# MrTornado24/FENeRF

Hardware: NVIDIA H100
Metric: rendered faces/sec at 128px x 24 samples/ray (higher is better)
Workload: dtype f16 operands / f32 accumulate (wgmma) + f32 refinement

## Files before the change

fenerf_b200/csrc/siren_fast.cu:

```cuda
#include "siren_fast.cuh"

namespace fn {

int siren_fast_label_launch(const void* args, int blocks, cudaStream_t st);
int siren_fast_hd_launch(const void* args, int blocks, bool label_film, cudaStream_t st);
int siren_fast_grid_launch(const void* args, int blocks, cudaStream_t st);
int siren_fast_bridge_launch(const void* args, int blocks, cudaStream_t st);
int siren_fast_debug_launch(const void* args, int blocks, bool label_film, bool feature_head, int variant, cudaStream_t st);

namespace {

std::atomic<int> g_variant{0};
unsigned long long* g_trace = nullptr;
int g_trace_ctas = 0;

bool build_loads(const FnLayout& L, FastArgs& A, bool sigma_only) {
    A.n_loads = 0;
    auto push = [&](size_t src, uint32_t bytes) {
        if (A.n_loads < MAX_LOADS) A.loads[A.n_loads] = Load{(uint32_t)src, bytes};
        ++A.n_loads;
    };
    push(L.first_img, 2 * CHUNK);
    if (L.grid_trunk) push(L.first_img_lo, 2 * CHUNK);
    for (int l = 0; l < L.n_hidden; ++l) {
        if (l == L.trunk_hidden) {
            push(L.head_img, 4 * HEAD_CHUNK);
            if (sigma_only) return A.n_loads <= MAX_LOADS;
        }
        if (L.bridge && l == L.color0) {
            push(L.color0_ximg, 2 * CHUNK);
            continue;
        }
        push(L.hid_img[l], 2 * CHUNK);
        push(L.hid_img[l] + 2 * CHUNK, 2 * CHUNK);
        if (l == L.label_layer) push(L.label.img, (uint32_t)FN_HEAD_IMG_BYTES(L.label.img_rows));
        if (l == L.color0) push(L.color0_ximg, 2 * CHUNK);
        push(L.hid_img[l] + 4 * CHUNK, 2 * CHUNK);
        push(L.hid_img[l] + 6 * CHUNK, 2 * CHUNK);
    }
    push(L.rgb.img, (uint32_t)FN_HEAD_IMG_BYTES(L.rgb.img_rows));
    return A.n_loads <= MAX_LOADS;
}

}

int siren_fast_debug_variant(int variant, unsigned long long* trace, int trace_ctas) {
    FN_REQUIRE(variant >= 0 && variant <= 3, "unknown point-network variant %d", variant);
    FN_REQUIRE(variant < 2 || (trace && trace_ctas >= 1), "a timeline variant needs its trace buffer");
    g_trace = trace;
    g_trace_ctas = trace_ctas;
    g_variant.store(variant);
    return 0;
}

int siren_points_fast(const FnLayout& L, const unsigned char* packed, const float* points, const float* dirs, const float* film,
                      int batch, long long ppb, int dir_group, int lock_dirs, float* out, int sigma_only, cudaStream_t st,
                      float* sigma_out) {
    static_assert(sizeof(FastArgs) <= 4000, "kernel parameter block too large");
    static_assert(SMEM_TOTAL <= 232448, "one CTA per SM: 227 KB of shared memory");
    static_assert(FN_HEAD_IMG_BYTES(FN_FEAT) == SLOT_BYTES, "a feature-head image is one ring slot");
    const bool trunk_only = L.feature_head && sigma_only;
    const bool feature_head = L.feature_head && !trunk_only, label_film = L.label_film && !trunk_only;
    FN_REQUIRE(L.trunk_hidden >= 1 && L.n_hidden - L.color0 >= 1, "field needs >= 2 trunk and >= 1 colour layers");
    FN_REQUIRE(L.sigma_row < 32, "the fast path packs labels and sigma into one 32-column head (label_dim <= 31)");
    FN_REQUIRE(L.rgb.img < 0xFFFFFFFFull && L.label.img < 0xFFFFFFFFull && L.first_img_lo < 0xFFFFFFFFull,
               "packed weight images beyond 4 GB");
    FN_REQUIRE(((uintptr_t)film & 15) == 0, "the FiLM table must be 16-byte aligned");
    if (L.wo_dir && !sigma_only)
        return fail(FENERF_E_UNSUPPORTED, "FENERF_FIELD_WO_DIR: the wgmma colour branch is not accurate for this field (its "
                    "first colour layer amplifies the fp16 trunk's error to ~2e-2 in rgb); render it with "
                    "FENERF_PRECISION_EXACT or FENERF_PRECISION_SPLIT (the density alone runs in any precision)");
    FastArgs a;
    memset(&a, 0, sizeof(a));
    FN_REQUIRE(build_loads(L, a, sigma_only != 0), "field too deep for the weight stream");
    a.sigma_only = sigma_only ? 1 : 0;
    a.L = L; a.packed = packed; a.points = points; a.dirs = dirs; a.film = film; a.out = out; a.sigma_out = sigma_out;
    a.ppb = ppb; a.tiles_per_batch = (ppb + TILE - 1) / TILE; a.n_tiles = a.tiles_per_batch * batch;
    a.dir_group = dir_group < 1 ? 1 : dir_group; a.lock_dirs = lock_dirs;
    if (a.n_tiles <= 0) return 0;
    FN_REQUIRE(ppb % a.dir_group == 0, "points_per_batch %lld not a multiple of dir_group %d", ppb, a.dir_group);
    const long long n_pairs = (a.n_tiles + 1) / 2;
    const int blocks = (int)(n_pairs < (long long)num_sms() ? n_pairs : (long long)num_sms());
    if (const int variant = g_variant.load()) {
        FN_REQUIRE(!L.grid_trunk && !L.bridge,
                   "the debug point-network variants do not cover fields with the grid in the trunk or a bridge");
        a.trace = g_trace;
        a.trace_ctas = g_trace_ctas;
        return siren_fast_debug_launch(&a, blocks, label_film, feature_head, variant, st);
    }
    if (L.grid_trunk) return siren_fast_grid_launch(&a, blocks, st);
    if (L.bridge) return siren_fast_bridge_launch(&a, blocks, st);
    if (feature_head) return siren_fast_hd_launch(&a, blocks, label_film, st);
    if (label_film) return siren_fast_label_launch(&a, blocks, st);
    return launch<siren_fast_kernel<false>>("siren_fast_kernel", blocks, NTHREADS, SMEM_TOTAL, st, a);
}

}
```

fenerf_b200/csrc/siren_fast.cuh:

```cuda
#pragma once
#include "common.cuh"
#include "siren_common.cuh"
#include "sm90.cuh"

namespace fn {

namespace {

using namespace sm90;

constexpr int TILE = 64;
constexpr int NTHREADS = 384;
constexpr int PROD_WARP = 8;
constexpr int RING = 6;
constexpr uint32_t SLOT_BYTES = 32768;
constexpr int XSTRIDE = 72;
constexpr uint32_t SMEM_X = RING * SLOT_BYTES;
constexpr int FRING = 2;
constexpr uint32_t FILM_BYTES = 2 * FN_H * 4;
constexpr uint32_t SMEM_FILM = SMEM_X + 2 * TILE * XSTRIDE * 2;
constexpr uint32_t SMEM_BAR = SMEM_FILM + 2 * FRING * FILM_BYTES;
constexpr uint32_t SMEM_TOTAL = SMEM_BAR + 16 * RING + 16 + 16 * 2 * FRING;
constexpr uint32_t SMEM_XLO = SMEM_TOTAL;
constexpr int XLO_STRIDE = 32;
constexpr uint32_t SMEM_TOTAL_GRID = SMEM_XLO + 2 * TILE * XLO_STRIDE * 2;
constexpr int RING_SPLIT = 4;
constexpr uint32_t ALO_CHUNK = TILE * FN_KCHUNK * 2;
constexpr uint32_t ALO_BYTES = (FN_H / FN_KCHUNK) * ALO_CHUNK;
constexpr uint32_t SPLIT_SMEM_ALO = RING_SPLIT * SLOT_BYTES;
constexpr uint32_t SPLIT_SMEM_X = SPLIT_SMEM_ALO + 2 * ALO_BYTES;
constexpr uint32_t SPLIT_SMEM_FILM = SPLIT_SMEM_X + 2 * TILE * XSTRIDE * 2;
constexpr uint32_t SPLIT_SMEM_BAR = SPLIT_SMEM_FILM + 2 * FRING * FILM_BYTES;
constexpr uint32_t SPLIT_SMEM_XLO = SPLIT_SMEM_BAR + 16 * RING_SPLIT + 16 + 16 * 2 * FRING;
constexpr uint32_t SMEM_TOTAL_SPLIT = SPLIT_SMEM_XLO + 2 * TILE * XLO_STRIDE * 2;
constexpr int MAX_LOADS = 72;
constexpr int MAX_LOADS_SPLIT = 132;
constexpr uint32_t CHUNK = 16384;
constexpr uint32_t HEAD_CHUNK = 32 * 128;
constexpr uint32_t RGB_CHUNK = 8 * 128;
constexpr uint32_t FEAT_CHUNK = FN_FEAT * 128;
#ifndef FENERF_SOFT_SIN_EVERY
#define FENERF_SOFT_SIN_EVERY 0
#endif
constexpr int kSoftSinEvery = FENERF_SOFT_SIN_EVERY;
constexpr int kSoftSinSplit = 4;
constexpr int TRACE_CAP = 1024;
constexpr int TRACE_WARPS = 11;
enum TraceEvent {
    TR_PAIR = 1, TR_TURN_WAIT, TR_TURN_DONE, TR_ACQ_WAIT, TR_ACQ_DONE, TR_COMMIT, TR_MMA_DONE, TR_EPI_DONE,
    TR_FILM_WAIT, TR_FILM_DONE, TR_EMPTY_WAIT, TR_EMPTY_DONE,
};
enum TraceGroup { TG_FIRST = 0, TG_HIDDEN, TG_COLOR0, TG_TRUNK_HEAD, TG_LABEL_LAYER, TG_LABEL_HEAD, TG_OUT_HEAD };

__device__ __forceinline__ float soft_sinf(float a) {
    const float k = fmaf(a, 0.159154943f, 12582912.f);
    const float n = k - 12582912.f;
    float r = fmaf(-n, 6.28318548f, a);
    r = fmaf(-n, -1.74845553e-7f, r);
    const float r2 = r * r;
    float p = -2.041572245e-08f;
    p = fmaf(p, r2, 2.701100129e-06f);
    p = fmaf(p, r2, -1.980991656e-04f);
    p = fmaf(p, r2, 8.332454599e-03f);
    p = fmaf(p, r2, -1.666656137e-01f);
    p = fmaf(p, r2, 9.999996424e-01f);
    return r * p;
}

struct Load {
    uint32_t src;
    uint32_t bytes;
};

template <int kMaxLoads>
struct FastArgsT {
    Load loads[kMaxLoads];
    int n_loads;
    FnLayout L;
    const unsigned char* packed;
    const float* points;
    const float* dirs;
    const float* film;
    float* out;
    float* sigma_out;
    long long ppb, tiles_per_batch, n_tiles;
    int dir_group, lock_dirs;
    int sigma_only;
    unsigned long long* trace;
    int trace_ctas;
};
using FastArgs = FastArgsT<MAX_LOADS>;
using SplitArgs = FastArgsT<MAX_LOADS_SPLIT>;

__device__ __forceinline__ void wg_bar(int wg) { asm volatile("bar.sync %0, 128;" ::"r"(1 + wg) : "memory"); }

template <bool kLabelFilm, bool kFeatureHead = false, int kSoftSin = kSoftSinEvery, bool kTrace = false,
          bool kGridTrunk = false, bool kBridge = false, bool kSplit = false>
__global__ void __launch_bounds__(NTHREADS, 1)
    siren_fast_kernel(const __grid_constant__ FastArgsT<kSplit ? MAX_LOADS_SPLIT : MAX_LOADS> a) {
    constexpr int RING = kSplit ? RING_SPLIT : fn::RING;
    constexpr uint32_t SMEM_X = kSplit ? SPLIT_SMEM_X : fn::SMEM_X;
    constexpr uint32_t SMEM_FILM = kSplit ? SPLIT_SMEM_FILM : fn::SMEM_FILM;
    constexpr uint32_t SMEM_BAR = kSplit ? SPLIT_SMEM_BAR : fn::SMEM_BAR;
    constexpr uint32_t SMEM_XLO = kSplit ? SPLIT_SMEM_XLO : fn::SMEM_XLO;
    extern __shared__ __align__(1024) unsigned char smem[];
    const uint32_t sbase = smem_u32(smem);
    const int warp = threadIdx.x >> 5, lane = threadIdx.x & 31;
    const uint32_t bar_full = sbase + SMEM_BAR, bar_empty = bar_full + 8 * RING, bar_turn = bar_empty + 8 * RING;
    const uint32_t bar_ffull = bar_turn + 16, bar_fempty = bar_ffull + 8 * 2 * FRING;
    unsigned long long* tbuf = nullptr;
    uint32_t tn = 0;
    if constexpr (kTrace)
        if (lane == 0 && (int)blockIdx.x < a.trace_ctas) tbuf = a.trace + ((size_t)blockIdx.x * TRACE_WARPS + warp) * TRACE_CAP;
    auto trace = [&](int kind, int group = 0) {
        if constexpr (kTrace)
            if (tbuf && tn < TRACE_CAP)
                tbuf[tn++] = ((unsigned long long)kind << 56) | ((unsigned long long)group << 48) |
                             ((unsigned long long)clock64() & ((1ull << 48) - 1));
    };
    if (threadIdx.x == 0) {
        for (int i = 0; i < RING; ++i) {
            mbar_init(bar_full + 8 * i, 1);
            mbar_init(bar_empty + 8 * i, 8);
        }
        for (int g = 0; g < 2; ++g) mbar_init(bar_turn + 8 * g, 4);
        for (int e = 0; e < 2 * FRING; ++e) {
            mbar_init(bar_ffull + 8 * e, 32);
            mbar_init(bar_fempty + 8 * e, 4);
        }
        fence_barrier_init();
    }
    __syncthreads();
    const long long n_pairs = (a.n_tiles + 1) / 2;

    if (warp >= PROD_WARP) {
        asm volatile("setmaxnreg.dec.sync.aligned.u32 40;\n" ::: "memory");
        if (warp == PROD_WARP && lane == 0) {
            uint32_t it = 0;
            for (long long pair = blockIdx.x; pair < n_pairs; pair += gridDim.x)
                for (int i = 0; i < a.n_loads; ++i, ++it) {
                    const uint32_t slot = it % RING;
                    trace(TR_EMPTY_WAIT);
                    mbar_wait(bar_empty + 8 * slot, ((it / RING) & 1u) ^ 1u);
                    trace(TR_EMPTY_DONE);
                    mbar_arrive_expect_tx(bar_full + 8 * slot, a.loads[i].bytes);
                    bulk_g2s(sbase + slot * SLOT_BYTES, a.packed + a.loads[i].src, a.loads[i].bytes, bar_full + 8 * slot);
                }
        } else if (warp == PROD_WARP + 1 || warp == PROD_WARP + 2) {
            const int g = warp - PROD_WARP - 1;
            const int n_film = 1 + (a.sigma_only ? a.L.trunk_hidden : a.L.n_hidden);
            uint32_t it = 0;
            for (long long pair = blockIdx.x; pair < n_pairs; pair += gridDim.x) {
                const long long tile = pair * 2 + g;
                const long long b = tile < a.n_tiles ? tile / a.tiles_per_batch : 0;
                const float* film_b = a.film + (size_t)b * a.L.n_film * 2 * FN_H;
                for (int i = 0; i < n_film; ++i, ++it) {
                    const uint32_t e = g * FRING + it % FRING;
                    const float2* row = reinterpret_cast<const float2*>(film_b + (size_t)i * 2 * FN_H);
                    const float2* bias = reinterpret_cast<const float2*>(a.packed + (i == 0 ? a.L.first_b : a.L.hid_b[i - 1]));
                    float4* dst = reinterpret_cast<float4*>(smem + SMEM_FILM + e * FILM_BYTES);
                    trace(TR_EMPTY_WAIT);
                    mbar_wait(bar_fempty + 8 * e, ((it / FRING) & 1u) ^ 1u);
                    trace(TR_EMPTY_DONE);
#pragma unroll 1
                    for (int k = 0; k < FN_H / 64; ++k) {
                        const int cp = lane + 32 * k;
                        const float2 f = __ldg(row + cp), p = __ldg(row + FN_H / 2 + cp), bb = __ldg(bias + cp);
                        if constexpr (kSplit) {
                            const float us = __ldg(reinterpret_cast<const float*>(a.packed + a.L.split_scale) +
                                                   FN_SPLIT_SCALES + i);
                            dst[cp] = make_float4(f.x * us, f.y * us, fmaf(f.x, bb.x, p.x), fmaf(f.y, bb.y, p.y));
                        } else {
                            dst[cp] = make_float4(f.x, f.y, fmaf(f.x, bb.x, p.x), fmaf(f.y, bb.y, p.y));
                        }
                    }
                    mbar_arrive(bar_ffull + 8 * e);
                }
            }
        }
        return;
    }

    asm volatile("setmaxnreg.inc.sync.aligned.u32 232;\n" ::: "memory");
    const int wg = warp >> 2, q = lane & 3;
    const int tid = threadIdx.x & 127;
    const int r0 = (warp & 3) * 16 + (lane >> 2);
    const FnLayout& L = a.L;
    const int C = L.out_dim;
    const float* sigma_w = reinterpret_cast<const float*>(a.packed + L.sigma_w);
    const float* label_w = reinterpret_cast<const float*>(a.packed + L.label_w);
    const int trunk_labels = (kLabelFilm || kFeatureHead) ? 0 : L.trunk_labels;
    const int sigma_row = kFeatureHead ? FN_FEAT_SIGMA_ROW : L.sigma_row;
    const int rgb_rows = kFeatureHead ? FN_FEAT : L.rgb.w_rows;
    const int label_rows = kFeatureHead ? FN_FEAT : L.label.w_rows;
    __half* xs = reinterpret_cast<__half*>(smem + SMEM_X) + wg * TILE * XSTRIDE;
    uint32_t it = 0;
    auto acquire = [&](uint32_t& slot) -> uint32_t {
        slot = it % RING;
        trace(TR_ACQ_WAIT);
        mbar_wait(bar_full + 8 * slot, (it / RING) & 1u);
        trace(TR_ACQ_DONE);
        ++it;
        return sbase + slot * SLOT_BYTES;
    };
    auto release = [&](uint32_t slot) {
        __syncwarp();
        if (lane == 0) mbar_arrive(bar_empty + 8 * slot);
    };
    uint32_t turns = 0;
    uint32_t fit = 0;
    auto film_acquire = [&]() -> const float4* {
        const uint32_t e = wg * FRING + fit % FRING;
        trace(TR_FILM_WAIT);
        mbar_wait(bar_ffull + 8 * e, (fit / FRING) & 1u);
        trace(TR_FILM_DONE);
        return reinterpret_cast<const float4*>(smem + SMEM_FILM + e * FILM_BYTES);
    };
    auto film_release = [&]() {
        const uint32_t e = wg * FRING + fit % FRING;
        ++fit;
        __syncwarp();
        if (lane == 0) mbar_arrive(bar_fempty + 8 * e);
    };
    auto turn_begin = [&]() {
        trace(TR_TURN_WAIT);
        mbar_wait(bar_turn + 8 * wg, (turns & 1u) ^ (wg == 0 ? 1u : 0u));
        trace(TR_TURN_DONE);
    };
    auto turn_end = [&](int group) {
        trace(TR_COMMIT, group);
        ++turns;
        __syncwarp();
        if (lane == 0) mbar_arrive(bar_turn + 8 * (wg ^ 1));
    };
    auto xfrag = [&](int s, uint32_t (&f)[4]) {
        const __half* p = xs + r0 * XSTRIDE + 16 * s + 2 * q;
        f[0] = *reinterpret_cast<const uint32_t*>(p);
        f[1] = *reinterpret_cast<const uint32_t*>(p + 8 * XSTRIDE);
        f[2] = *reinterpret_cast<const uint32_t*>(p + 8);
        f[3] = *reinterpret_cast<const uint32_t*>(p + 8 * XSTRIDE + 8);
    };

    for (long long pair = blockIdx.x; pair < n_pairs; pair += gridDim.x) {
        const long long tile = pair * 2 + wg;
        const bool tile_ok = tile < a.n_tiles;
        const long long b = tile_ok ? tile / a.tiles_per_batch : 0;
        const long long p0 = tile_ok ? (tile % a.tiles_per_batch) * TILE : a.ppb;
        trace(TR_PAIR);

        wg_bar(wg);
        if (tid < TILE) {
            float pos[3] = {0.f, 0.f, 0.f}, dir[3] = {0.f, 0.f, 0.f};
            const long long pp = p0 + tid;
            const bool valid = pp < a.ppb;
            if (valid) {
                const long long ff = b * a.ppb + pp;
#pragma unroll
                for (int i = 0; i < 3; ++i) pos[i] = __fmul_rn(a.points[ff * 3 + i], L.input_scale);
                if (a.lock_dirs) dir[2] = -1.f;
                else {
                    const long long di = b * (a.ppb / a.dir_group) + pp / a.dir_group;
#pragma unroll
                    for (int i = 0; i < 3; ++i) dir[i] = a.dirs[di * 3 + i];
                }
            }
            __align__(16) __half slots[64];
#pragma unroll
            for (int i = 0; i < 64; ++i) slots[i] = __float2half_rn(0.f);
#pragma unroll
            for (int i = 0; i < 3; ++i) {
                __half hi, lo;
                split_f16(pos[i], hi, lo);
                slots[FN_SLOT_POS + i] = hi; slots[FN_SLOT_POS + 3 + i] = lo; slots[FN_SLOT_POS + 6 + i] = hi;
                split_f16(dir[i], hi, lo);
                slots[FN_SLOT_DIR + i] = hi; slots[FN_SLOT_DIR + 3 + i] = lo; slots[FN_SLOT_DIR + 6 + i] = hi;
            }
            if constexpr (kGridTrunk || kSplit) {
                __align__(16) __half lo[32];
#pragma unroll
                for (int i = 0; i < 32; ++i) lo[i] = __float2half_rn(0.f);
                if (valid && (kGridTrunk || (L.grid_channels > 0 && !a.sigma_only))) {
                    float feat[32];
                    grid_features32(reinterpret_cast<const float*>(a.packed + L.grid), L.grid_res, pos[0], pos[1], pos[2], feat);
#pragma unroll
                    for (int i = 0; i < 32; ++i) split_f16(feat[i], slots[FN_SLOT_FEAT + i], lo[i]);
                }
                __half* xlo = reinterpret_cast<__half*>(smem + SMEM_XLO) + (wg * TILE + tid) * XLO_STRIDE;
#pragma unroll
                for (int i = 0; i < 4; ++i) reinterpret_cast<uint4*>(xlo)[i] = reinterpret_cast<const uint4*>(lo)[i];
            } else if (L.grid_channels > 0 && valid && !a.sigma_only) {
                float feat[32];
                grid_features32_h(reinterpret_cast<const __half*>(a.packed + L.grid16), L.grid_res, pos[0], pos[1], pos[2], feat);
#pragma unroll
                for (int i = 0; i < 32; ++i) slots[FN_SLOT_FEAT + i] = __float2half_rn(feat[i]);
            }
#pragma unroll
            for (int i = 0; i < 8; ++i)
                reinterpret_cast<uint4*>(xs + tid * XSTRIDE)[i] = reinterpret_cast<const uint4*>(slots)[i];
        }
        wg_bar(wg);

        uint32_t act[16][4];
        uint32_t nxt[8][4];
        float d[64];
        auto film_epi = [&](const float4* fs, int h, uint32_t (&dst)[8][4]) {
#pragma unroll
            for (int j = 0; j < 16; ++j) {
                const float4 e = fs[64 * h + 4 * j + q];
                const bool soft = kSoftSin > 0 && j % (kSoftSin > 0 ? kSoftSin : 1) == kSoftSin - 1;
                auto sn = [soft](float x) { return soft ? soft_sinf(x) : __sinf(x); };
                dst[j >> 1][(j & 1) * 2] = pack_half2(sn(fmaf(e.x, d[4 * j], e.z)), sn(fmaf(e.y, d[4 * j + 1], e.w)));
                dst[j >> 1][(j & 1) * 2 + 1] = pack_half2(sn(fmaf(e.x, d[4 * j + 2], e.z)), sn(fmaf(e.y, d[4 * j + 3], e.w)));
            }
            trace(TR_EPI_DONE);
        };
        auto act_hi = [&]() -> uint32_t (&)[8][4] { return *reinterpret_cast<uint32_t (*)[8][4]>(&act[8]); };
        auto film_epi_split = [&](const float4* fs, int h, uint32_t (&dst)[8][4], uint32_t (&lo)[8][4]) {
#pragma unroll
            for (int j = 0; j < 16; ++j) {
                const float4 e = fs[64 * h + 4 * j + q];
#pragma unroll
                for (int rr = 0; rr < 2; ++rr) {
                    const float s0 = soft_sinf(fmaf(e.x, d[4 * j + 2 * rr], e.z));
                    const float s1 = soft_sinf(fmaf(e.y, d[4 * j + 2 * rr + 1], e.w));
                    const __half2 hi = __floats2half2_rn(s0, s1);
                    const float2 hf = __half22float2(hi);
                    dst[j >> 1][(j & 1) * 2 + rr] = *reinterpret_cast<const uint32_t*>(&hi);
                    lo[j >> 1][(j & 1) * 2 + rr] = pack_half2(s0 - hf.x, s1 - hf.y);
                }
            }
            trace(TR_EPI_DONE);
        };
        const uint32_t alo_base = sbase + SPLIT_SMEM_ALO + wg * ALO_BYTES;
        auto alo_desc = [&](int s) { return desc_kmajor(alo_base + (s >> 2) * ALO_CHUNK + 32 * (s & 3)); };
        auto alo_store = [&](const uint32_t (&lo0)[8][4], const uint32_t (&lo1)[8][4]) {
            wg_bar(wg);
            unsigned char* base = smem + SPLIT_SMEM_ALO + wg * ALO_BYTES;
#pragma unroll
            for (int h = 0; h < 2; ++h)
#pragma unroll
                for (int j = 0; j < 16; ++j) {
                    const int col = 128 * h + 8 * j + 2 * q;
#pragma unroll
                    for (int rr = 0; rr < 2; ++rr)
                        *reinterpret_cast<uint32_t*>(base + (col >> 6) * ALO_CHUNK + fn_sw128_offset(r0 + 8 * rr, col & 63)) =
                            (h ? lo1 : lo0)[j >> 1][(j & 1) * 2 + rr];
                }
            fence_async_smem();
            wg_bar(wg);
        };
        uint32_t lo0[8][4], lo1[8][4];

        {
            uint32_t xf[4], slot, slot_lo = 0, w_lo = 0;
            uint32_t xg[2][4], xl[2][4];
            const float4* fs = nullptr;
            xfrag(0, xf);
            if constexpr (kGridTrunk) {
                const __half* xlo = reinterpret_cast<const __half*>(smem + SMEM_XLO) + wg * TILE * XLO_STRIDE;
#pragma unroll
                for (int s = 0; s < 2; ++s) {
                    xfrag(2 + s, xg[s]);
                    const __half* p = xlo + r0 * XLO_STRIDE + 16 * s + 2 * q;
                    xl[s][0] = *reinterpret_cast<const uint32_t*>(p);
                    xl[s][1] = *reinterpret_cast<const uint32_t*>(p + 8 * XLO_STRIDE);
                    xl[s][2] = *reinterpret_cast<const uint32_t*>(p + 8);
                    xl[s][3] = *reinterpret_cast<const uint32_t*>(p + 8 * XLO_STRIDE + 8);
                }
            }
            const uint32_t w = acquire(slot);
            if constexpr (kGridTrunk) w_lo = acquire(slot_lo);
#pragma unroll
            for (int h = 0; h < 2; ++h) {
                turn_begin();
                wg_fence();
                mma_rs_n128(d, xf, desc_kmajor(w + h * CHUNK), 0u);
                if constexpr (kGridTrunk)
#pragma unroll
                    for (int s = 0; s < 2; ++s) {
                        mma_rs_n128(d, xg[s], desc_kmajor(w + h * CHUNK + 32 * (2 + s)), 1u);
                        mma_rs_n128(d, xl[s], desc_kmajor(w + h * CHUNK + 32 * (2 + s)), 1u);
                        mma_rs_n128(d, xg[s], desc_kmajor(w_lo + h * CHUNK + 32 * (2 + s)), 1u);
                    }
                wg_commit();
                turn_end(TG_FIRST);
                wg_wait<0>();
                trace(TR_MMA_DONE);
                fence_regs(d);
                fence_regs(xf);
                if constexpr (kGridTrunk) { fence_regs(xg); fence_regs(xl); }
                if (h == 0) fs = film_acquire();
                if constexpr (kSplit) {
                    if (h == 0) film_epi_split(fs, 0, nxt, lo0);
                    else film_epi_split(fs, 1, act_hi(), lo1);
                } else {
                    if (h == 0) film_epi(fs, 0, nxt);
                    else film_epi(fs, 1, act_hi());
                }
            }
            release(slot);
            if constexpr (kGridTrunk) release(slot_lo);
            film_release();
            if constexpr (kSplit) alo_store(lo0, lo1);
#pragma unroll
            for (int s = 0; s < 8; ++s)
#pragma unroll
                for (int i = 0; i < 4; ++i) act[s][i] = nxt[s][i];
        }

        bool stop = false;
        for (int l = 0; l < L.n_hidden && !stop; ++l) {
            if (l == L.trunk_hidden) {
                float dh[16];
                uint32_t slot, slot_lo = 0, w_lo = 0;
                const uint32_t w = acquire(slot);
                if constexpr (kSplit) w_lo = acquire(slot_lo);
                turn_begin();
                wg_fence();
#pragma unroll
                for (int c = 0; c < 4; ++c)
#pragma unroll
                    for (int k = 0; k < 4; ++k) mma_rs_n32(dh, act[4 * c + k], desc_kmajor(w + c * HEAD_CHUNK + 32 * k), (c | k) ? 1u : 0u);
                if constexpr (kSplit)
#pragma unroll
                    for (int c = 0; c < 4; ++c)
#pragma unroll
                        for (int k = 0; k < 4; ++k) {
                            mma_ss_n32(dh, alo_desc(4 * c + k), desc_kmajor(w + c * HEAD_CHUNK + 32 * k), 1u);
                            mma_rs_n32(dh, act[4 * c + k], desc_kmajor(w_lo + c * HEAD_CHUNK + 32 * k), 1u);
                        }
                wg_commit();
                turn_end(TG_TRUNK_HEAD);
                wg_wait<0>();
                trace(TR_MMA_DONE);
                fence_regs(dh);
                fence_regs(act);
                release(slot);
                if constexpr (kSplit) {
                    release(slot_lo);
                    const float us = __ldg(reinterpret_cast<const float*>(a.packed + L.split_scale) + FN_SPLIT_SCALES +
                                           L.n_hidden + 1);
#pragma unroll
                    for (int i = 0; i < 16; ++i) dh[i] *= us;
                }
                const float* lb = label_w + FENERF_MAX_LABEL * FN_H;
#pragma unroll
                for (int rr = 0; rr < 2; ++rr) {
                    const long long pnt = p0 + r0 + 8 * rr;
                    if (pnt >= a.ppb) continue;
                    const long long flat = b * a.ppb + pnt;
#pragma unroll
                    for (int i = 0; i < 4; ++i)
#pragma unroll
                        for (int e = 0; e < 2; ++e) {
                            const int o = 8 * i + 2 * q + e;
                            const float v = dh[4 * i + 2 * rr + e];
                            if (o < trunk_labels) {
                                if (!a.sigma_only) a.out[flat * C + o] = fmaf(v, __ldg(lb + FENERF_MAX_LABEL), __ldg(lb + o));
                            } else if (o == sigma_row && !(kBridge && L.bridge_res)) {
                                const float sig = v + __ldg(sigma_w + FN_H);
                                a.out[flat * C + (C - 1)] = sig;
                                if (a.sigma_out) a.sigma_out[flat] = sig;
                            }
                        }
                }
                if constexpr (kBridge) {
                    const float* bw = reinterpret_cast<const float*>(a.packed + L.bridge_w);
#pragma unroll
                    for (int rr = 0; rr < 2; ++rr) {
                        const float o0 = dh[2 * rr], o1 = dh[2 * rr + 1];
                        const float p2 = __shfl_xor_sync(0xffffffffu, o0, 1), p3 = __shfl_xor_sync(0xffffffffu, o1, 1);
                        if (q != 0) continue;
                        const long long pnt = p0 + r0 + 8 * rr;
                        float v[3] = {o1 + __ldg(bw + 3 * FN_H), p2 + __ldg(bw + 3 * FN_H + 1), p3 + __ldg(bw + 3 * FN_H + 2)};
                        if (L.bridge_res) {
                            if (pnt < a.ppb) {
                                const long long flat = b * a.ppb + pnt;
#pragma unroll
                                for (int j = 0; j < 3; ++j) v[j] += __fmul_rn(a.points[flat * 3 + j], L.input_scale);
                                float sig = __ldg(bw + 3 * FN_H + 6);
#pragma unroll
                                for (int j = 0; j < 3; ++j) sig = fmaf(__ldg(bw + 3 * FN_H + 3 + j), v[j], sig);
                                a.out[flat * C + (C - 1)] = sig;
                                if (a.sigma_out) a.sigma_out[flat] = sig;
                            }
                        }
                        if (!a.sigma_only) {
                            __half* row = xs + (r0 + 8 * rr) * XSTRIDE + FN_SLOT_FEAT;
#pragma unroll
                            for (int j = 0; j < 3; ++j) {
// ... 71 lines not shown
                    }
                    continue;
                }
            }
            const bool c0 = (l == L.color0);
            if constexpr (kSplit) {
                const bool grid = L.grid_channels > 0;
                const float4* fs = nullptr;
#pragma unroll
                for (int h = 0; h < 2; ++h) {
                    uint32_t sl[4], w[4];
#pragma unroll
                    for (int i = 0; i < 4; ++i) w[i] = acquire(sl[i]);
                    turn_begin();
                    wg_fence();
#pragma unroll
                    for (int s = 0; s < 16; ++s)
                        mma_rs_n128(d, act[s], desc_kmajor(w[s >> 3] + ((s >> 2) & 1) * CHUNK + 32 * (s & 3)), s ? 1u : 0u);
#pragma unroll
                    for (int s = 0; s < 16; ++s)
                        mma_ss_n128(d, alo_desc(s), desc_kmajor(w[s >> 3] + ((s >> 2) & 1) * CHUNK + 32 * (s & 3)), 1u);
#pragma unroll
                    for (int s = 0; s < 16; ++s)
                        mma_rs_n128(d, act[s], desc_kmajor(w[2 + (s >> 3)] + ((s >> 2) & 1) * CHUNK + 32 * (s & 3)), 1u);
                    wg_commit();
                    turn_end(c0 ? TG_COLOR0 : TG_HIDDEN);
                    wg_wait<0>();
                    trace(TR_MMA_DONE);
                    fence_regs(d);
                    fence_regs(act);
#pragma unroll
                    for (int i = 0; i < 4; ++i) release(sl[i]);
                    if (c0) {
                        uint32_t xf[3][4], xl[2][4], slot_x, slot_xl = 0, w_xl = 0;
#pragma unroll
                        for (int s = 0; s < 3; ++s) xfrag(1 + s, xf[s]);
                        const __half* xlo = reinterpret_cast<const __half*>(smem + SMEM_XLO) + wg * TILE * XLO_STRIDE;
#pragma unroll
                        for (int s = 0; s < 2; ++s) {
                            const __half* p = xlo + r0 * XLO_STRIDE + 16 * s + 2 * q;
                            xl[s][0] = *reinterpret_cast<const uint32_t*>(p);
                            xl[s][1] = *reinterpret_cast<const uint32_t*>(p + 8 * XLO_STRIDE);
                            xl[s][2] = *reinterpret_cast<const uint32_t*>(p + 8);
                            xl[s][3] = *reinterpret_cast<const uint32_t*>(p + 8 * XLO_STRIDE + 8);
                        }
                        const uint32_t w_x = acquire(slot_x);
                        if (grid) w_xl = acquire(slot_xl);
                        turn_begin();
                        wg_fence();
                        mma_rs_n128(d, xf[0], desc_kmajor(w_x + h * CHUNK + 32), 1u);
                        if (grid)
#pragma unroll
                            for (int s = 0; s < 2; ++s) {
                                const uint32_t off = h * CHUNK + 32 * (2 + s);
                                mma_rs_n128(d, xf[1 + s], desc_kmajor(w_x + off), 1u);
                                mma_rs_n128(d, xl[s], desc_kmajor(w_x + off), 1u);
                                mma_rs_n128(d, xf[1 + s], desc_kmajor(w_xl + off), 1u);
                            }
                        wg_commit();
                        turn_end(TG_COLOR0);
                        wg_wait<0>();
                        trace(TR_MMA_DONE);
                        fence_regs(d);
                        fence_regs(xf);
                        fence_regs(xl);
                        release(slot_x);
                        if (grid) release(slot_xl);
                    }
                    if (h == 0) fs = film_acquire();
                    if (h == 0) film_epi_split(fs, 0, nxt, lo0);
                    else film_epi_split(fs, 1, act_hi(), lo1);
                }
                film_release();
                alo_store(lo0, lo1);
#pragma unroll
                for (int s = 0; s < 8; ++s)
#pragma unroll
                    for (int i = 0; i < 4; ++i) act[s][i] = nxt[s][i];
                continue;
            }
            const bool narrow = kBridge && c0;
            const int nx = kBridge ? 2 : !kGridTrunk && L.grid_channels > 0 ? 3 : 1;
            uint32_t xf[3][4];
            if (c0)
#pragma unroll
                for (int s = 0; s < 3; ++s) xfrag(1 + s, xf[s]);
            uint32_t slot_x = 0, w_x = 0;
            const float4* fs = nullptr;
#pragma unroll
            for (int h = 0; h < 2; ++h) {
                uint32_t sl[2] = {0u, 0u};
                if (narrow && h == 0) w_x = acquire(slot_x);
                turn_begin();
                wg_fence();
                if (!narrow)
#pragma unroll
                    for (int sb = 0; sb < 2; ++sb) {
                        const uint32_t w = acquire(sl[sb]);
#pragma unroll
                        for (int c = 0; c < 2; ++c)
#pragma unroll
                            for (int k = 0; k < 4; ++k)
                                mma_rs_n128(d, act[8 * sb + 4 * c + k], desc_kmajor(w + c * CHUNK + 32 * k), (sb | c | k) ? 1u : 0u);
                    }
                if (c0) {
                    if (h == 0 && !narrow) w_x = acquire(slot_x);
#pragma unroll
                    for (int s = 0; s < 3; ++s)
                        if (s < nx) mma_rs_n128(d, xf[s], desc_kmajor(w_x + h * CHUNK + 32 * (1 + s)), (narrow && s == 0) ? 0u : 1u);
                }
                wg_commit();
                turn_end(c0 ? TG_COLOR0 : TG_HIDDEN);
                wg_wait<0>();
                trace(TR_MMA_DONE);
                fence_regs(d);
                fence_regs(act);
                fence_regs(xf);
                if (!narrow) {
                    release(sl[0]);
                    release(sl[1]);
                }
                if (c0 && h == 1) release(slot_x);
                if (h == 0) fs = film_acquire();
                if (h == 0) film_epi(fs, 0, nxt);
                else film_epi(fs, 1, act_hi());
            }
            film_release();
#pragma unroll
            for (int s = 0; s < 8; ++s)
#pragma unroll
                for (int i = 0; i < 4; ++i) act[s][i] = nxt[s][i];
        }
        if (stop) continue;

        if constexpr (kFeatureHead) {
            float dr[32];
            uint32_t slot;
            const uint32_t w = acquire(slot);
            turn_begin();
            wg_fence();
#pragma unroll
            for (int c = 0; c < 4; ++c)
#pragma unroll
                for (int k = 0; k < 4; ++k) mma_rs_n64(dr, act[4 * c + k], desc_kmajor(w + c * FEAT_CHUNK + 32 * k), (c | k) ? 1u : 0u);
            wg_commit();
            turn_end(TG_OUT_HEAD);
            wg_wait<0>();
            trace(TR_MMA_DONE);
            fence_regs(dr);
            fence_regs(act);
            release(slot);
            const float* rgb_b = reinterpret_cast<const float*>(a.packed + L.rgb.w) + rgb_rows * FN_H;
#pragma unroll
            for (int rr = 0; rr < 2; ++rr) {
                const long long pnt = p0 + r0 + 8 * rr;
                if (pnt >= a.ppb) continue;
                const long long flat = b * a.ppb + pnt;
#pragma unroll
                for (int i = 0; i < 8; ++i)
#pragma unroll
                    for (int e = 0; e < 2; ++e) {
                        const int o = 8 * i + 2 * q + e;
                        a.out[flat * C + L.label_dim + o] = dr[4 * i + 2 * rr + e] + __ldg(rgb_b + o);
                    }
            }
            continue;
        }
        {
            float dr[4];
            uint32_t slot, slot_lo = 0, w_lo = 0;
            const uint32_t w = acquire(slot);
            if constexpr (kSplit) w_lo = acquire(slot_lo);
            turn_begin();
            wg_fence();
#pragma unroll
            for (int c = 0; c < 4; ++c)
#pragma unroll
                for (int k = 0; k < 4; ++k) mma_rs_n8(dr, act[4 * c + k], desc_kmajor(w + c * RGB_CHUNK + 32 * k), (c | k) ? 1u : 0u);
            if constexpr (kSplit)
#pragma unroll
                for (int c = 0; c < 4; ++c)
#pragma unroll
                    for (int k = 0; k < 4; ++k) {
                        mma_ss_n8(dr, alo_desc(4 * c + k), desc_kmajor(w + c * RGB_CHUNK + 32 * k), 1u);
                        mma_rs_n8(dr, act[4 * c + k], desc_kmajor(w_lo + c * RGB_CHUNK + 32 * k), 1u);
                    }
            wg_commit();
            turn_end(TG_OUT_HEAD);
            wg_wait<0>();
            trace(TR_MMA_DONE);
            fence_regs(dr);
            fence_regs(act);
            release(slot);
            if constexpr (kSplit) {
                release(slot_lo);
                const float us = __ldg(reinterpret_cast<const float*>(a.packed + L.split_scale) + FN_SPLIT_SCALES +
                                       L.n_hidden + 2);
#pragma unroll
                for (int i = 0; i < 4; ++i) dr[i] *= us;
            }
            const float* rgb_b = reinterpret_cast<const float*>(a.packed + L.rgb.w) + rgb_rows * FN_H;
#pragma unroll
            for (int rr = 0; rr < 2; ++rr) {
                const long long pnt = p0 + r0 + 8 * rr;
                if (pnt >= a.ppb) continue;
                const long long flat = b * a.ppb + pnt;
#pragma unroll
                for (int e = 0; e < 2; ++e) {
                    const int o = 2 * q + e;
                    if (o < 3) {
                        const float x = dr[2 * rr + e] + __ldg(rgb_b + o);
                        a.out[flat * C + L.label_dim + o] = __fdividef(1.f, 1.f + __expf(-x));
                    }
                }
// ... 9 lines not shown
```

fenerf_b200/csrc/siren_fast_debug.cu:

```cuda
#include "siren_fast.cuh"

namespace fn {

namespace {

template <bool kLabelFilm, bool kFeatureHead, int kSoftSin, bool kTrace>
int debug_launch(const FastArgs& a, int blocks, cudaStream_t st) {
    return launch<siren_fast_kernel<kLabelFilm, kFeatureHead, kSoftSin, kTrace>>("siren_fast_kernel<debug>", blocks, NTHREADS,
                                                                                SMEM_TOTAL, st, a);
}

__global__ void soft_sine_kernel(const float* a, float* out, long long n) {
    const long long i = (long long)blockIdx.x * blockDim.x + threadIdx.x;
    if (i < n) out[i] = soft_sinf(a[i]);
}

}

int siren_fast_debug_launch(const void* args, int blocks, bool label_film, bool feature_head, int variant, cudaStream_t st) {
    const FastArgs& a = *static_cast<const FastArgs*>(args);
    if (variant == 1) {
        if (feature_head) return label_film ? debug_launch<true, true, kSoftSinSplit, false>(a, blocks, st) : debug_launch<false, true, kSoftSinSplit, false>(a, blocks, st);
        return label_film ? debug_launch<true, false, kSoftSinSplit, false>(a, blocks, st) : debug_launch<false, false, kSoftSinSplit, false>(a, blocks, st);
    }
    FN_REQUIRE(!label_film && !feature_head, "the point-network timeline covers plain fields only");
    if (variant == 2) return debug_launch<false, false, kSoftSinEvery, true>(a, blocks, st);
    return debug_launch<false, false, kSoftSinSplit, true>(a, blocks, st);
}

int soft_sine_eval(const float* a, float* out, long long n, cudaStream_t st) {
    if (n <= 0) return 0;
    soft_sine_kernel<<<(unsigned)((n + 255) / 256), 256, 0, st>>>(a, out, n);
    FN_LAUNCH_OK("soft_sine_kernel");
    return 0;
}

}
```

fenerf_b200/csrc/siren_fast_hd.cu:

```cuda
#include "siren_fast.cuh"

namespace fn {

int siren_fast_hd_launch(const void* args, int blocks, bool label_film, cudaStream_t st) {
    const FastArgs& a = *static_cast<const FastArgs*>(args);
    if (label_film)
        return launch<siren_fast_kernel<true, true>>("siren_fast_kernel<label FiLM, feature head>", blocks, NTHREADS,
                                                     SMEM_TOTAL, st, a);
    return launch<siren_fast_kernel<false, true>>("siren_fast_kernel<feature head>", blocks, NTHREADS, SMEM_TOTAL, st, a);
}

}
```

Baseline: 594.9.

## Run three consumer warpgroups per CTA for plain and feature-head SIREN kernels

Adds a three-consumer-warpgroup variant of the warp-specialized SIREN kernel for plain and feature-head fields. Each CTA now handles three 64-point tiles per turn instead of two, so more independent MMA streams share one weight stream. To fit the smaller register budget (160 per consumer thread), the input is kept in swizzled shared memory and fed to wgmma as an SS operand, and half of the next-layer activations is parked in shared memory between halves. The ring shrinks to four slots, and tile indices switch to 32-bit with a new size guard. The cost is more shared-memory traffic and a shallower weight prefetch.

```diff
diff --git a/fenerf_b200/csrc/siren_fast.cu b/fenerf_b200/csrc/siren_fast.cu
--- a/fenerf_b200/csrc/siren_fast.cu
+++ b/fenerf_b200/csrc/siren_fast.cu
@@ -3,10 +3,10 @@
 namespace fn {
 
 int siren_fast_label_launch(const void* args, int blocks, cudaStream_t st);
-int siren_fast_hd_launch(const void* args, int blocks, bool label_film, cudaStream_t st);
+int siren_fast_hd_launch(const void* args, bool label_film, cudaStream_t st);
 int siren_fast_grid_launch(const void* args, int blocks, cudaStream_t st);
 int siren_fast_bridge_launch(const void* args, int blocks, cudaStream_t st);
-int siren_fast_debug_launch(const void* args, int blocks, bool label_film, bool feature_head, int variant, cudaStream_t st);
+int siren_fast_debug_launch(const void* args, bool label_film, bool feature_head, int variant, cudaStream_t st);
 
 namespace {
 
@@ -57,7 +57,7 @@
                       int batch, long long ppb, int dir_group, int lock_dirs, float* out, int sigma_only, cudaStream_t st,
                       float* sigma_out) {
     static_assert(sizeof(FastArgs) <= 4000, "kernel parameter block too large");
-    static_assert(SMEM_TOTAL <= 232448, "one CTA per SM: 227 KB of shared memory");
+    static_assert(SMEM_TOTAL <= 232448 && SMEM3_TOTAL <= 232448, "one CTA per SM: 227 KB of shared memory");
     static_assert(FN_HEAD_IMG_BYTES(FN_FEAT) == SLOT_BYTES, "a feature-head image is one ring slot");
     const bool trunk_only = L.feature_head && sigma_only;
     const bool feature_head = L.feature_head && !trunk_only, label_film = L.label_film && !trunk_only;
@@ -79,20 +79,24 @@
     a.dir_group = dir_group < 1 ? 1 : dir_group; a.lock_dirs = lock_dirs;
     if (a.n_tiles <= 0) return 0;
     FN_REQUIRE(ppb % a.dir_group == 0, "points_per_batch %lld not a multiple of dir_group %d", ppb, a.dir_group);
-    const long long n_pairs = (a.n_tiles + 1) / 2;
-    const int blocks = (int)(n_pairs < (long long)num_sms() ? n_pairs : (long long)num_sms());
+    if (!L.grid_trunk && !L.bridge && !label_film)
+        FN_REQUIRE(a.n_tiles < (1ll << 31) - WG_PLAIN && ppb < (1ll << 31) - TILE,
+                   "the fast point network indexes tiles and points in 32 bits: %lld tiles of 64 points over the batch "
+                   "(at most 2^31 - %d), %lld points per image (at most 2^31 - %d)", a.n_tiles, WG_PLAIN + 1, ppb, TILE + 1);
     if (const int variant = g_variant.load()) {
         FN_REQUIRE(!L.grid_trunk && !L.bridge,
                    "the debug point-network variants do not cover fields with the grid in the trunk or a bridge");
         a.trace = g_trace;
         a.trace_ctas = g_trace_ctas;
-        return siren_fast_debug_launch(&a, blocks, label_film, feature_head, variant, st);
+        return siren_fast_debug_launch(&a, label_film, feature_head, variant, st);
     }
+    const int blocks = fast_ctas(a.n_tiles, 2);
     if (L.grid_trunk) return siren_fast_grid_launch(&a, blocks, st);
     if (L.bridge) return siren_fast_bridge_launch(&a, blocks, st);
-    if (feature_head) return siren_fast_hd_launch(&a, blocks, label_film, st);
+    if (feature_head) return siren_fast_hd_launch(&a, label_film, st);
     if (label_film) return siren_fast_label_launch(&a, blocks, st);
-    return launch<siren_fast_kernel<false>>("siren_fast_kernel", blocks, NTHREADS, SMEM_TOTAL, st, a);
+    return launch<siren_fast_kernel<false, false, kSoftSinEvery, false, false, false, false, WG_PLAIN>>(
+        "siren_fast_kernel", fast_ctas(a.n_tiles, WG_PLAIN), fast_threads(WG_PLAIN), fast_smem(WG_PLAIN), st, a);
 }
 
 }
diff --git a/fenerf_b200/csrc/siren_fast.cuh b/fenerf_b200/csrc/siren_fast.cuh
--- a/fenerf_b200/csrc/siren_fast.cuh
+++ b/fenerf_b200/csrc/siren_fast.cuh
@@ -25,6 +25,18 @@
 constexpr int XLO_STRIDE = 32;
 constexpr uint32_t SMEM_TOTAL_GRID = SMEM_XLO + 2 * TILE * XLO_STRIDE * 2;
 constexpr int RING_SPLIT = 4;
+constexpr int WG_PLAIN = 3;
+constexpr int RING3 = 4;
+constexpr uint32_t PARK_BYTES = 128 * 8 * 16;
+constexpr uint32_t X3_BYTES = TILE * 64 * 2;
+constexpr uint32_t SMEM3_PARK = RING3 * SLOT_BYTES;
+constexpr uint32_t SMEM3_X = SMEM3_PARK + 3 * PARK_BYTES;
+constexpr uint32_t SMEM3_FILM = SMEM3_X + 3 * X3_BYTES;
+constexpr uint32_t SMEM3_BAR = SMEM3_FILM + 3 * FRING * FILM_BYTES;
+constexpr uint32_t SMEM3_TOTAL = SMEM3_BAR + 16 * RING3 + 8 * 3 + 16 * 3 * FRING;
+static_assert(SMEM3_TOTAL == 217272 && SMEM3_X % 1024 == 0, "three warpgroups: the shared-memory plan");
+constexpr int fast_threads(int wgs) { return 128 * (wgs + 1); }
+constexpr uint32_t fast_smem(int wgs) { return wgs == 3 ? SMEM3_TOTAL : SMEM_TOTAL; }
 constexpr uint32_t ALO_CHUNK = TILE * FN_KCHUNK * 2;
 constexpr uint32_t ALO_BYTES = (FN_H / FN_KCHUNK) * ALO_CHUNK;
 constexpr uint32_t SPLIT_SMEM_ALO = RING_SPLIT * SLOT_BYTES;
@@ -45,7 +57,7 @@
 constexpr int kSoftSinEvery = FENERF_SOFT_SIN_EVERY;
 constexpr int kSoftSinSplit = 4;
 constexpr int TRACE_CAP = 1024;
-constexpr int TRACE_WARPS = 11;
+constexpr int TRACE_WARPS = 16;
 enum TraceEvent {
     TR_PAIR = 1, TR_TURN_WAIT, TR_TURN_DONE, TR_ACQ_WAIT, TR_ACQ_DONE, TR_COMMIT, TR_MMA_DONE, TR_EPI_DONE,
     TR_FILM_WAIT, TR_FILM_DONE, TR_EMPTY_WAIT, TR_EMPTY_DONE,
@@ -94,50 +106,59 @@
 
 __device__ __forceinline__ void wg_bar(int wg) { asm volatile("bar.sync %0, 128;" ::"r"(1 + wg) : "memory"); }
 
+inline int fast_ctas(long long n_tiles, int wgs) {
+    const long long n_groups = (n_tiles + wgs - 1) / wgs;
+    return (int)(n_groups < (long long)num_sms() ? n_groups : (long long)num_sms());
+}
+
 template <bool kLabelFilm, bool kFeatureHead = false, int kSoftSin = kSoftSinEvery, bool kTrace = false,
-          bool kGridTrunk = false, bool kBridge = false, bool kSplit = false>
-__global__ void __launch_bounds__(NTHREADS, 1)
+          bool kGridTrunk = false, bool kBridge = false, bool kSplit = false, int kWG = 2>
+__global__ void __launch_bounds__(fast_threads(kWG), 1)
     siren_fast_kernel(const __grid_constant__ FastArgsT<kSplit ? MAX_LOADS_SPLIT : MAX_LOADS> a) {
-    constexpr int RING = kSplit ? RING_SPLIT : fn::RING;
-    constexpr uint32_t SMEM_X = kSplit ? SPLIT_SMEM_X : fn::SMEM_X;
-    constexpr uint32_t SMEM_FILM = kSplit ? SPLIT_SMEM_FILM : fn::SMEM_FILM;
-    constexpr uint32_t SMEM_BAR = kSplit ? SPLIT_SMEM_BAR : fn::SMEM_BAR;
+    static_assert(kWG == 2 || (kWG == 3 && !kSplit), "two consumer warpgroups, or three without the A_lo regions");
+    constexpr int RING = kSplit ? RING_SPLIT : kWG == 3 ? RING3 : fn::RING;
+    constexpr int PROD_WARP = 4 * kWG;
+    constexpr uint32_t SMEM_X = kSplit ? SPLIT_SMEM_X : kWG == 3 ? SMEM3_X : fn::SMEM_X;
+    constexpr uint32_t SMEM_FILM = kSplit ? SPLIT_SMEM_FILM : kWG == 3 ? SMEM3_FILM : fn::SMEM_FILM;
+    constexpr uint32_t SMEM_BAR = kSplit ? SPLIT_SMEM_BAR : kWG == 3 ? SMEM3_BAR : fn::SMEM_BAR;
     constexpr uint32_t SMEM_XLO = kSplit ? SPLIT_SMEM_XLO : fn::SMEM_XLO;
     extern __shared__ __align__(1024) unsigned char smem[];
     const uint32_t sbase = smem_u32(smem);
     const int warp = threadIdx.x >> 5, lane = threadIdx.x & 31;
     const uint32_t bar_full = sbase + SMEM_BAR, bar_empty = bar_full + 8 * RING, bar_turn = bar_empty + 8 * RING;
-    const uint32_t bar_ffull = bar_turn + 16, bar_fempty = bar_ffull + 8 * 2 * FRING;
-    unsigned long long* tbuf = nullptr;
-    uint32_t tn = 0;
+    const uint32_t bar_ffull = bar_turn + 8 * kWG, bar_fempty = bar_ffull + 8 * kWG * FRING;
+    uint32_t tn = TRACE_CAP;
     if constexpr (kTrace)
-        if (lane == 0 && (int)blockIdx.x < a.trace_ctas) tbuf = a.trace + ((size_t)blockIdx.x * TRACE_WARPS + warp) * TRACE_CAP;
+        if (lane == 0 && (int)blockIdx.x < a.trace_ctas) tn = 0;
     auto trace = [&](int kind, int group = 0) {
         if constexpr (kTrace)
-            if (tbuf && tn < TRACE_CAP)
-                tbuf[tn++] = ((unsigned long long)kind << 56) | ((unsigned long long)group << 48) |
-                             ((unsigned long long)clock64() & ((1ull << 48) - 1));
+            if (tn < TRACE_CAP)
+                a.trace[((size_t)blockIdx.x * TRACE_WARPS + (threadIdx.x >> 5)) * TRACE_CAP + tn++] =
+                    ((unsigned long long)kind << 56) | ((unsigned long long)group << 48) |
+                    ((unsigned long long)clock64() & ((1ull << 48) - 1));
     };
     if (threadIdx.x == 0) {
         for (int i = 0; i < RING; ++i) {
             mbar_init(bar_full + 8 * i, 1);
-            mbar_init(bar_empty + 8 * i, 8);
+            mbar_init(bar_empty + 8 * i, 4 * kWG);
         }
-        for (int g = 0; g < 2; ++g) mbar_init(bar_turn + 8 * g, 4);
-        for (int e = 0; e < 2 * FRING; ++e) {
+        for (int g = 0; g < kWG; ++g) mbar_init(bar_turn + 8 * g, 4);
+        for (int e = 0; e < kWG * FRING; ++e) {
             mbar_init(bar_ffull + 8 * e, 32);
             mbar_init(bar_fempty + 8 * e, 4);
         }
         fence_barrier_init();
     }
     __syncthreads();
-    const long long n_pairs = (a.n_tiles + 1) / 2;
+    using Idx = std::conditional_t<kWG == 3, int, long long>;
+    const Idx n_groups = (Idx)((a.n_tiles + kWG - 1) / kWG);
 
     if (warp >= PROD_WARP) {
-        asm volatile("setmaxnreg.dec.sync.aligned.u32 40;\n" ::: "memory");
+        if constexpr (kWG == 3) asm volatile("setmaxnreg.dec.sync.aligned.u32 32;\n" ::: "memory");
+        else asm volatile("setmaxnreg.dec.sync.aligned.u32 40;\n" ::: "memory");
         if (warp == PROD_WARP && lane == 0) {
             uint32_t it = 0;
-            for (long long pair = blockIdx.x; pair < n_pairs; pair += gridDim.x)
+            for (Idx grp = blockIdx.x; grp < n_groups; grp += gridDim.x)
                 for (int i = 0; i < a.n_loads; ++i, ++it) {
                     const uint32_t slot = it % RING;
                     trace(TR_EMPTY_WAIT);
@@ -146,13 +167,13 @@
                     mbar_arrive_expect_tx(bar_full + 8 * slot, a.loads[i].bytes);
                     bulk_g2s(sbase + slot * SLOT_BYTES, a.packed + a.loads[i].src, a.loads[i].bytes, bar_full + 8 * slot);
                 }
-        } else if (warp == PROD_WARP + 1 || warp == PROD_WARP + 2) {
+        } else if (warp == PROD_WARP + 1 || warp == PROD_WARP + 2 || (kWG == 3 && warp == PROD_WARP + 3)) {
             const int g = warp - PROD_WARP - 1;
             const int n_film = 1 + (a.sigma_only ? a.L.trunk_hidden : a.L.n_hidden);
             uint32_t it = 0;
-            for (long long pair = blockIdx.x; pair < n_pairs; pair += gridDim.x) {
-                const long long tile = pair * 2 + g;
-                const long long b = tile < a.n_tiles ? tile / a.tiles_per_batch : 0;
+            for (Idx grp = blockIdx.x; grp < n_groups; grp += gridDim.x) {
+                const Idx tile = grp * kWG + g;
+                const Idx b = tile < a.n_tiles ? tile / a.tiles_per_batch : 0;
                 const float* film_b = a.film + (size_t)b * a.L.n_film * 2 * FN_H;
                 for (int i = 0; i < n_film; ++i, ++it) {
                     const uint32_t e = g * FRING + it % FRING;
@@ -181,7 +202,8 @@
         return;
     }
 
-    asm volatile("setmaxnreg.inc.sync.aligned.u32 232;\n" ::: "memory");
+    if constexpr (kWG == 3) asm volatile("setmaxnreg.inc.sync.aligned.u32 160;\n" ::: "memory");
+    else asm volatile("setmaxnreg.inc.sync.aligned.u32 232;\n" ::: "memory");
     const int wg = warp >> 2, q = lane & 3;
     const int tid = threadIdx.x & 127;
     const int r0 = (warp & 3) * 16 + (lane >> 2);
@@ -194,6 +216,8 @@
     const int rgb_rows = kFeatureHead ? FN_FEAT : L.rgb.w_rows;
     const int label_rows = kFeatureHead ? FN_FEAT : L.label.w_rows;
     __half* xs = reinterpret_cast<__half*>(smem + SMEM_X) + wg * TILE * XSTRIDE;
+    unsigned char* const xs3 = smem + SMEM_X + wg * X3_BYTES;
+    const uint32_t xs3_addr = sbase + SMEM_X + wg * X3_BYTES;
     uint32_t it = 0;
     auto acquire = [&](uint32_t& slot) -> uint32_t {
         slot = it % RING;
@@ -208,6 +232,7 @@
         if (lane == 0) mbar_arrive(bar_empty + 8 * slot);
     };
     uint32_t turns = 0;
+    const int next_wg = kWG == 2 ? (wg ^ 1) : (wg + 1) % kWG;
     uint32_t fit = 0;
     auto film_acquire = [&]() -> const float4* {
         const uint32_t e = wg * FRING + fit % FRING;
@@ -231,7 +256,7 @@
         trace(TR_COMMIT, group);
         ++turns;
         __syncwarp();
-        if (lane == 0) mbar_arrive(bar_turn + 8 * (wg ^ 1));
+        if (lane == 0) mbar_arrive(bar_turn + 8 * next_wg);
     };
     auto xfrag = [&](int s, uint32_t (&f)[4]) {
         const __half* p = xs + r0 * XSTRIDE + 16 * s + 2 * q;
@@ -241,11 +266,11 @@
         f[3] = *reinterpret_cast<const uint32_t*>(p + 8 * XSTRIDE + 8);
     };
 
-    for (long long pair = blockIdx.x; pair < n_pairs; pair += gridDim.x) {
-        const long long tile = pair * 2 + wg;
+    for (Idx grp = blockIdx.x; grp < n_groups; grp += gridDim.x) {
+        const Idx tile = grp * kWG + wg;
         const bool tile_ok = tile < a.n_tiles;
-        const long long b = tile_ok ? tile / a.tiles_per_batch : 0;
-        const long long p0 = tile_ok ? (tile % a.tiles_per_batch) * TILE : a.ppb;
+        const Idx b = tile_ok ? tile / a.tiles_per_batch : 0;
+        const Idx p0 = tile_ok ? (tile % a.tiles_per_batch) * TILE : a.ppb;
         trace(TR_PAIR);
 
         wg_bar(wg);
@@ -294,9 +319,16 @@
 #pragma unroll
                 for (int i = 0; i < 32; ++i) slots[FN_SLOT_FEAT + i] = __float2half_rn(feat[i]);
             }
-#pragma unroll
-            for (int i = 0; i < 8; ++i)
-                reinterpret_cast<uint4*>(xs + tid * XSTRIDE)[i] = reinterpret_cast<const uint4*>(slots)[i];
+            if constexpr (kWG == 3) {
+#pragma unroll
+                for (int i = 0; i < 8; ++i)
+                    *reinterpret_cast<uint4*>(xs3 + fn_sw128_offset(tid, 8 * i)) = reinterpret_cast<const uint4*>(slots)[i];
+                fence_async_smem();
+            } else {
+#pragma unroll
+                for (int i = 0; i < 8; ++i)
+                    reinterpret_cast<uint4*>(xs + tid * XSTRIDE)[i] = reinterpret_cast<const uint4*>(slots)[i];
+            }
         }
         wg_bar(wg);
 
@@ -315,6 +347,22 @@
             trace(TR_EPI_DONE);
         };
         auto act_hi = [&]() -> uint32_t (&)[8][4] { return *reinterpret_cast<uint32_t (*)[8][4]>(&act[8]); };
+        uint4* const park = reinterpret_cast<uint4*>(smem + SMEM3_PARK + wg * PARK_BYTES) + tid;
+        auto park_store = [&]() {
+            if constexpr (kWG == 3) {
+#pragma unroll
+                for (int s = 0; s < 8; ++s) park[128 * s] = make_uint4(nxt[s][0], nxt[s][1], nxt[s][2], nxt[s][3]);
+            }
+        };
+        auto park_load = [&]() {
+            if constexpr (kWG == 3) {
+#pragma unroll
+                for (int s = 0; s < 8; ++s) {
+                    const uint4 v = park[128 * s];
+                    act[s][0] = v.x; act[s][1] = v.y; act[s][2] = v.z; act[s][3] = v.w;
+                }
+            }
+        };
         auto film_epi_split = [&](const float4* fs, int h, uint32_t (&dst)[8][4], uint32_t (&lo)[8][4]) {
 #pragma unroll
             for (int j = 0; j < 16; ++j) {
@@ -355,7 +403,7 @@
             uint32_t xf[4], slot, slot_lo = 0, w_lo = 0;
             uint32_t xg[2][4], xl[2][4];
             const float4* fs = nullptr;
-            xfrag(0, xf);
+            if constexpr (kWG == 2) xfrag(0, xf);
             if constexpr (kGridTrunk) {
                 const __half* xlo = reinterpret_cast<const __half*>(smem + SMEM_XLO) + wg * TILE * XLO_STRIDE;
 #pragma unroll
@@ -374,7 +422,8 @@
             for (int h = 0; h < 2; ++h) {
                 turn_begin();
                 wg_fence();
-                mma_rs_n128(d, xf, desc_kmajor(w + h * CHUNK), 0u);
+                if constexpr (kWG == 3) mma_ss_n128(d, desc_kmajor(xs3_addr), desc_kmajor(w + h * CHUNK), 0u);
+                else mma_rs_n128(d, xf, desc_kmajor(w + h * CHUNK), 0u);
                 if constexpr (kGridTrunk)
 #pragma unroll
                     for (int s = 0; s < 2; ++s) {
@@ -387,25 +436,27 @@
                 wg_wait<0>();
                 trace(TR_MMA_DONE);
                 fence_regs(d);
-                fence_regs(xf);
+                if constexpr (kWG == 2) fence_regs(xf);
                 if constexpr (kGridTrunk) { fence_regs(xg); fence_regs(xl); }
                 if (h == 0) fs = film_acquire();
                 if constexpr (kSplit) {
                     if (h == 0) film_epi_split(fs, 0, nxt, lo0);
                     else film_epi_split(fs, 1, act_hi(), lo1);
                 } else {
-                    if (h == 0) film_epi(fs, 0, nxt);
-                    else film_epi(fs, 1, act_hi());
+                    if (h == 0) { film_epi(fs, 0, nxt); park_store(); }
+                    else { park_load(); film_epi(fs, 1, act_hi()); }
                 }
             }
             release(slot);
             if constexpr (kGridTrunk) release(slot_lo);
             film_release();
             if constexpr (kSplit) alo_store(lo0, lo1);
-#pragma unroll
-            for (int s = 0; s < 8; ++s)
-#pragma unroll
-                for (int i = 0; i < 4; ++i) act[s][i] = nxt[s][i];
+            if constexpr (kWG == 2) {
+#pragma unroll
+                for (int s = 0; s < 8; ++s)
+#pragma unroll
+                    for (int i = 0; i < 4; ++i) act[s][i] = nxt[s][i];
+            }
         }
 
         bool stop = false;
@@ -643,9 +694,11 @@
             const bool narrow = kBridge && c0;
             const int nx = kBridge ? 2 : !kGridTrunk && L.grid_channels > 0 ? 3 : 1;
             uint32_t xf[3][4];
-            if (c0)
-#pragma unroll
-                for (int s = 0; s < 3; ++s) xfrag(1 + s, xf[s]);
+            if constexpr (kWG == 2) {
+                if (c0)
+#pragma unroll
+                    for (int s = 0; s < 3; ++s) xfrag(1 + s, xf[s]);
+            }
             uint32_t slot_x = 0, w_x = 0;
             const float4* fs = nullptr;
 #pragma unroll
@@ -668,7 +721,11 @@
                     if (h == 0 && !narrow) w_x = acquire(slot_x);
 #pragma unroll
                     for (int s = 0; s < 3; ++s)
-                        if (s < nx) mma_rs_n128(d, xf[s], desc_kmajor(w_x + h * CHUNK + 32 * (1 + s)), (narrow && s == 0) ? 0u : 1u);
+                        if (s < nx) {
+                            const uint64_t wd = desc_kmajor(w_x + h * CHUNK + 32 * (1 + s));
+                            if constexpr (kWG == 3) mma_ss_n128(d, desc_kmajor(xs3_addr + 32 * (1 + s)), wd, (narrow && s == 0) ? 0u : 1u);
+                            else mma_rs_n128(d, xf[s], wd, (narrow && s == 0) ? 0u : 1u);
+                        }
                 }
                 wg_commit();
                 turn_end(c0 ? TG_COLOR0 : TG_HIDDEN);
@@ -676,21 +733,23 @@
                 trace(TR_MMA_DONE);
                 fence_regs(d);
                 fence_regs(act);
-                fence_regs(xf);
+                if constexpr (kWG == 2) fence_regs(xf);
                 if (!narrow) {
                     release(sl[0]);
                     release(sl[1]);
                 }
                 if (c0 && h == 1) release(slot_x);
                 if (h == 0) fs = film_acquire();
-                if (h == 0) film_epi(fs, 0, nxt);
-                else film_epi(fs, 1, act_hi());
+                if (h == 0) { film_epi(fs, 0, nxt); park_store(); }
+                else { park_load(); film_epi(fs, 1, act_hi()); }
             }
             film_release();
-#pragma unroll
-            for (int s = 0; s < 8; ++s)
-#pragma unroll
-                for (int i = 0; i < 4; ++i) act[s][i] = nxt[s][i];
+            if constexpr (kWG == 2) {
+#pragma unroll
+                for (int s = 0; s < 8; ++s)
+#pragma unroll
+                    for (int i = 0; i < 4; ++i) act[s][i] = nxt[s][i];
+            }
         }
         if (stop) continue;
 
diff --git a/fenerf_b200/csrc/siren_fast_debug.cu b/fenerf_b200/csrc/siren_fast_debug.cu
--- a/fenerf_b200/csrc/siren_fast_debug.cu
+++ b/fenerf_b200/csrc/siren_fast_debug.cu
@@ -5,9 +5,10 @@
 namespace {
 
 template <bool kLabelFilm, bool kFeatureHead, int kSoftSin, bool kTrace>
-int debug_launch(const FastArgs& a, int blocks, cudaStream_t st) {
-    return launch<siren_fast_kernel<kLabelFilm, kFeatureHead, kSoftSin, kTrace>>("siren_fast_kernel<debug>", blocks, NTHREADS,
-                                                                                SMEM_TOTAL, st, a);
+int debug_launch(const FastArgs& a, cudaStream_t st) {
+    constexpr int kWG = kLabelFilm ? 2 : WG_PLAIN;
+    return launch<siren_fast_kernel<kLabelFilm, kFeatureHead, kSoftSin, kTrace, false, false, false, kWG>>(
+        "siren_fast_kernel<debug>", fast_ctas(a.n_tiles, kWG), fast_threads(kWG), fast_smem(kWG), st, a);
 }
 
 __global__ void soft_sine_kernel(const float* a, float* out, long long n) {
@@ -17,15 +18,15 @@
 
 }
 
-int siren_fast_debug_launch(const void* args, int blocks, bool label_film, bool feature_head, int variant, cudaStream_t st) {
+int siren_fast_debug_launch(const void* args, bool label_film, bool feature_head, int variant, cudaStream_t st) {
     const FastArgs& a = *static_cast<const FastArgs*>(args);
     if (variant == 1) {
-        if (feature_head) return label_film ? debug_launch<true, true, kSoftSinSplit, false>(a, blocks, st) : debug_launch<false, true, kSoftSinSplit, false>(a, blocks, st);
-        return label_film ? debug_launch<true, false, kSoftSinSplit, false>(a, blocks, st) : debug_launch<false, false, kSoftSinSplit, false>(a, blocks, st);
+        if (feature_head) return label_film ? debug_launch<true, true, kSoftSinSplit, false>(a, st) : debug_launch<false, true, kSoftSinSplit, false>(a, st);
+        return label_film ? debug_launch<true, false, kSoftSinSplit, false>(a, st) : debug_launch<false, false, kSoftSinSplit, false>(a, st);
     }
     FN_REQUIRE(!label_film && !feature_head, "the point-network timeline covers plain fields only");
-    if (variant == 2) return debug_launch<false, false, kSoftSinEvery, true>(a, blocks, st);
-    return debug_launch<false, false, kSoftSinSplit, true>(a, blocks, st);
+    if (variant == 2) return debug_launch<false, false, kSoftSinEvery, true>(a, st);
+    return debug_launch<false, false, kSoftSinSplit, true>(a, st);
 }
 
 int soft_sine_eval(const float* a, float* out, long long n, cudaStream_t st) {
diff --git a/fenerf_b200/csrc/siren_fast_hd.cu b/fenerf_b200/csrc/siren_fast_hd.cu
--- a/fenerf_b200/csrc/siren_fast_hd.cu
+++ b/fenerf_b200/csrc/siren_fast_hd.cu
@@ -2,12 +2,13 @@
 
 namespace fn {
 
-int siren_fast_hd_launch(const void* args, int blocks, bool label_film, cudaStream_t st) {
+int siren_fast_hd_launch(const void* args, bool label_film, cudaStream_t st) {
     const FastArgs& a = *static_cast<const FastArgs*>(args);
     if (label_film)
-        return launch<siren_fast_kernel<true, true>>("siren_fast_kernel<label FiLM, feature head>", blocks, NTHREADS,
-                                                     SMEM_TOTAL, st, a);
-    return launch<siren_fast_kernel<false, true>>("siren_fast_kernel<feature head>", blocks, NTHREADS, SMEM_TOTAL, st, a);
+        return launch<siren_fast_kernel<true, true>>("siren_fast_kernel<label FiLM, feature head>", fast_ctas(a.n_tiles, 2),
+                                                     NTHREADS, SMEM_TOTAL, st, a);
+    return launch<siren_fast_kernel<false, true, kSoftSinEvery, false, false, false, false, WG_PLAIN>>(
+        "siren_fast_kernel<feature head>", fast_ctas(a.n_tiles, WG_PLAIN), fast_threads(WG_PLAIN), fast_smem(WG_PLAIN), st, a);
 }
 
 }
```

Result: faster. 653.4, median of 6 (+9.8%).
